# hwang595/ATOMO

Measured on NVIDIA H100. Metric: ResNet-18 CIFAR-10 images/sec (whole box, device-timed, max over ranks), higher is better.
Workload: dtype bf16

## Files before the change

atomo_b200/csrc/bindings.cpp:

```cpp
#include <ATen/cuda/CUDAContext.h>
#include <c10/cuda/CUDAGuard.h>
#include <torch/extension.h>

#include <cstdint>
#include <string>

extern "C" {
const char* atomo_heap_last_error();
int atomo_heap_multicast_supported(int device);
int atomo_heap_posix_fd_supported(int device);
void* atomo_heap_create_vmm(int rank, int world, int device, size_t bytes, const char* job, int want_mc,
                            double timeout_s);
int atomo_heap_mc_phase_a(void* h, double timeout_s);
int atomo_heap_mc_phase_b(void* h);
void* atomo_heap_create_ipc(int rank, int world, int device, size_t bytes, unsigned char* handle_out64);
int atomo_heap_open_ipc(void* h, const unsigned char* all_handles);
uint64_t atomo_heap_ptr(void* h, int rank);
uint64_t atomo_heap_mc_ptr(void* h);
uint64_t atomo_heap_bytes(void* h);
const char* atomo_heap_mode(void* h);
void atomo_heap_destroy(void* h);
void atomo_launch_gram(const float* grad, const void* layers, const void* tiles, int ntiles, float* gpart,
                       cudaStream_t stream);
void atomo_launch_eig_sample(const void* layers, const int* ts_layers, int n_ts, const float* gpart, float* vsel,
                             int* selcount, float* sigma_out, float* ps_arena_peer, long long arena_floats,
                             const void* ctrl, const float* ext_uniforms, int rank, int random_sample,
                             int waterfill, int systematic, int worker_index, int threads, cudaStream_t stream);
void atomo_launch_project_push(const float* grad, const void* layers, const void* tiles, int ntiles,
                               const float* vsel, const int* selcount, float* ps_arena_peer,
                               long long arena_floats, int* push_flag_peer, void* ctrl, int worker_index,
                               int signal, cudaStream_t stream);
void atomo_launch_signal_push(int* push_flag_peer, const void* ctrl, int worker_index, cudaStream_t stream);
int atomo_ps_smem_bytes();
int atomo_ps_tile_elems();
int atomo_ps_max_rows();
int atomo_ps_dense_elems();
int atomo_ps_max_workers();
void atomo_launch_ps_update(const void* layers, const void* tiles, int ntiles, int W, int nflags, int nranks,
                            float* params, float* momentum, float* const* params_peer, float* params_mc,
                            const float* const* grads_peer, const float* grads_mc, const float* arenas,
                            long long arena_floats, int* push_flags, int* const* param_flag_peer, void* ctrl,
                            long long timeout_ticks, float inv_w, int grid, long long* tstats, cudaStream_t stream);
void atomo_launch_wait_params(const int* param_flag, void* ctrl, long long timeout_ticks, long long* tstats,
                              cudaStream_t stream);
void atomo_launch_advance_step(void* ctrl, cudaStream_t stream);
void atomo_launch_param_bcast(const float* src, float* const* params_peer, float* params_mc, int nranks,
                              int self_rank, long long numel, cudaStream_t stream);
void atomo_launch_set_flags(int* const* flag_peer, int nranks, int value, cudaStream_t stream);
long long atomo_bn_partial_floats(long long R, int C);
void atomo_launch_bn_forward(const void* x, const void* res, void* y, long long R, int C, float* acc, float* part,
                             const float* gamma, const float* beta, float* save_mean, float* save_invstd,
                             float* running_mean, float* running_var, float eps, float momentum, int relu,
                             cudaStream_t stream);
void atomo_launch_bn_backward(const void* dy, const void* x, const void* y, void* dx, void* dres, long long R, int C,
                              const float* mean, const float* invstd, const float* gamma, float* acc, float* part,
                              float* dgamma, float* dbeta, int relu, cudaStream_t stream);
int atomo_v2_unit_bytes();
int atomo_v2_ctrl_bytes();
int atomo_v2_enc_smem();
int atomo_v2_ps_smem();
int atomo_v2_ps_tile_elems();
void atomo_v2_launch_encode(const void* units, const void* tiles, int tile0, int ntiles, const long long* gptr,
                            float* gpart, unsigned int* unit_counters, float* vsel, int* selcount, float* sigma_out,
                            float* const* arena_peer, int n_owners, long long arena_floats, void* stage,
                            const void* ctrl, const float* ext_uniforms, float* vprev, int max_sweeps,
                            int random_sample, int waterfill, int systematic, int worker, int resample_empty,
                            int flags, long long* tstats, int group, cudaStream_t stream);
void atomo_v2_launch_project(const void* units, const void* tiles, int tile0, int ntiles, const long long* gptr,
                             const float* vsel, const int* selcount, float* const* arena_peer, int* const* sig_peer,
                             int n_owners, long long arena_floats, int worker, int group, void* ctrl,
                             unsigned int* group_counter, int flags, long long* tstats, int final_group, int timed,
                             cudaStream_t stream);
void atomo_v2_launch_ps(const void* units, const void* tiles, int tile0, int ntiles, int W, int nranks, int group,
                        int final_group, int owner, float* master, float* mom, float* sq, float* sqmax, float* vmom,
                        float* vsq, float* vsqmax, void* wshadow_mc, void* const* wshadow_peer, float* vparams_local,
                        float* vparams_mc, float* const* vparams_peer, const float* vgrads_mc,
                        const float* const* vgrads_peer, const void* const* stage_peer, const float* arenas,
                        long long arena_floats, int* sig, int* const* sig_peer, void* ctrl,
                        unsigned int* group_counter, long long timeout, long long* tstats, float inv_w, int grid,
                        cudaStream_t stream);
void atomo_v2_launch_wait_params(const int* sig, int n_owners, void* ctrl, long long timeout, long long* tstats,
                                 cudaStream_t stream);
void atomo_v2_launch_advance_step(void* ctrl, cudaStream_t stream);
void atomo_v2_launch_bcast_bytes(const void* src, void* const* peer, void* mc, int nranks, int self, long long nbytes,
                                 cudaStream_t stream);
int atomo_gemm_tile_bytes();
int atomo_gemm_smem_bytes();
void atomo_launch_skinny_gemm(const void* tiles, int ntiles, void* ctrl, int grid, cudaStream_t stream);
void atomo_launch_ext_finalize(const void* descs, const void* tiles, int ntiles, const float* arena_y,
                               const float* arena_b, float* ps_arena_peer, long long arena_floats,
                               const void* ctrl, int worker_index, cudaStream_t stream);
int atomo_ext_desc_bytes();
void atomo_launch_qsgd_encode(const float* grad, long long numel, int bucket, int q, int terngrad,
                              const float* clip_ptr, unsigned long long* words_out, float* norms_out,
                              const void* ctrl, int worker_index, const float* ext_uniforms, cudaStream_t stream);
void atomo_launch_qsgd_decode_sum(const unsigned long long* const* words, const float* const* norms, int W,
                                  long long numel, int bucket, int q, int terngrad, float* out_sum,
                                  const int* push_flags, void* ctrl, long long timeout_ticks, cudaStream_t stream);
int atomo_qsgd_max_bucket();
void atomo_launch_entrywise_encode(const float* grad, const void* layers, const void* tiles, int ntiles, float* l1,
                                   int nlayers, float budget, int* idx_out, float* val_out, int* count_out,
                                   int capacity, int* local_count, int* push_flag_peer, void* ctrl,
                                   int worker_index, const float* ext_uniforms, int signal, cudaStream_t stream);
void atomo_launch_entrywise_scatter(const int* const* idx, const float* const* val, const int* const* count, int W,
                                    int capacity, float* out_sum, long long numel, const int* push_flags,
                                    void* ctrl, long long timeout_ticks, cudaStream_t stream);
}

namespace {

inline cudaStream_t cur_stream() { return at::cuda::getCurrentCUDAStream().stream(); }
template <typename T>
inline T* P(uint64_t v) { return reinterpret_cast<T*>(static_cast<uintptr_t>(v)); }

void check_cuda_f32(const torch::Tensor& t, const char* name) {
  TORCH_CHECK(t.is_cuda(), name, " must be a CUDA tensor");
  TORCH_CHECK(t.scalar_type() == torch::kFloat32, name, " must be float32");
  TORCH_CHECK(t.is_contiguous(), name, " must be contiguous");
}

uint64_t heap_create_vmm(int rank, int world, int device, uint64_t bytes, const std::string& job, bool want_mc,
                         double timeout_s) {
  void* h = atomo_heap_create_vmm(rank, world, device, bytes, job.c_str(), want_mc ? 1 : 0, timeout_s);
  return reinterpret_cast<uint64_t>(h);
}
py::tuple heap_create_ipc(int rank, int world, int device, uint64_t bytes) {
  unsigned char handle[64] = {0};
  void* h = atomo_heap_create_ipc(rank, world, device, bytes, handle);
  return py::make_tuple(reinterpret_cast<uint64_t>(h), py::bytes(reinterpret_cast<const char*>(handle), 64));
}
bool heap_open_ipc(uint64_t h, const std::string& all_handles) {
  return atomo_heap_open_ipc(P<void>(h), reinterpret_cast<const unsigned char*>(all_handles.data())) != 0;
}

torch::Tensor tensor_from_ptr(uint64_t ptr, int64_t numel, const std::string& dtype, int device) {
  auto dt = dtype == "int32"      ? torch::kInt32
            : dtype == "int64"    ? torch::kInt64
            : dtype == "uint8"    ? torch::kUInt8
            : dtype == "bfloat16" ? torch::kBFloat16
                                  : torch::kFloat32;
  auto opts = torch::TensorOptions().dtype(dt).device(torch::kCUDA, device);
  return torch::from_blob(P<void>(ptr), {numel}, [](void*) {}, opts);
}

void gram(const torch::Tensor& grad, const torch::Tensor& layers, const torch::Tensor& tiles, int ntiles,
          torch::Tensor gpart) {
  check_cuda_f32(grad, "grad");
  c10::cuda::CUDAGuard guard(grad.device());
  atomo_launch_gram(grad.data_ptr<float>(), layers.data_ptr(), tiles.data_ptr(), ntiles, gpart.data_ptr<float>(),
                    cur_stream());
}

void eig_sample(const torch::Tensor& layers, const torch::Tensor& ts_layers, const torch::Tensor& gpart,
                torch::Tensor vsel, torch::Tensor selcount, c10::optional<torch::Tensor> sigma_out,
                uint64_t ps_arena_peer, int64_t arena_floats, const torch::Tensor& ctrl,
                c10::optional<torch::Tensor> ext_uniforms, int rank, bool random_sample, bool waterfill,
                bool systematic, int worker_index, int threads) {
  c10::cuda::CUDAGuard guard(gpart.device());
  atomo_launch_eig_sample(layers.data_ptr(), ts_layers.data_ptr<int>(), (int)ts_layers.numel(),
                          gpart.data_ptr<float>(), vsel.data_ptr<float>(), selcount.data_ptr<int>(),
                          sigma_out.has_value() ? sigma_out->data_ptr<float>() : nullptr, P<float>(ps_arena_peer),
                          arena_floats, ctrl.data_ptr(),
                          ext_uniforms.has_value() ? ext_uniforms->data_ptr<float>() : nullptr, rank,
                          random_sample, waterfill, systematic, worker_index, threads, cur_stream());
}

void project_push(const torch::Tensor& grad, const torch::Tensor& layers, const torch::Tensor& tiles, int ntiles,
                  const torch::Tensor& vsel, const torch::Tensor& selcount, uint64_t ps_arena_peer,
                  int64_t arena_floats, uint64_t push_flag_peer, torch::Tensor ctrl, int worker_index, bool signal) {
  check_cuda_f32(grad, "grad");
  c10::cuda::CUDAGuard guard(grad.device());
  atomo_launch_project_push(grad.data_ptr<float>(), layers.data_ptr(), tiles.data_ptr(), ntiles,
                            vsel.data_ptr<float>(), selcount.data_ptr<int>(), P<float>(ps_arena_peer), arena_floats,
                            P<int>(push_flag_peer), ctrl.data_ptr(), worker_index, signal ? 1 : 0, cur_stream());
}

void signal_push(uint64_t push_flag_peer, const torch::Tensor& ctrl, int worker_index) {
  c10::cuda::CUDAGuard guard(ctrl.device());
  atomo_launch_signal_push(P<int>(push_flag_peer), ctrl.data_ptr(), worker_index, cur_stream());
}

void check_nhwc_bf16(const torch::Tensor& t, const char* name) {
  TORCH_CHECK(t.is_cuda() && t.scalar_type() == torch::kBFloat16, name, " must be a CUDA bf16 tensor");
  TORCH_CHECK(t.dim() == 4 && t.is_contiguous(at::MemoryFormat::ChannelsLast), name, " must be channels_last");
  TORCH_CHECK(t.size(1) % 8 == 0 && t.size(1) <= 2048, name, ": C must be a multiple of 8 (<= 2048)");
}

void bn_forward(const torch::Tensor& x, c10::optional<torch::Tensor> res, torch::Tensor y, torch::Tensor acc,
                const torch::Tensor& gamma, const torch::Tensor& beta, torch::Tensor save_mean,
                torch::Tensor save_invstd, c10::optional<torch::Tensor> running_mean,
                c10::optional<torch::Tensor> running_var, double eps, double momentum, bool relu) {
  check_nhwc_bf16(x, "x");
  check_nhwc_bf16(y, "y");
  if (res.has_value()) check_nhwc_bf16(*res, "residual");
  c10::cuda::CUDAGuard guard(x.device());
  const long long R = x.numel() / x.size(1);
  auto part = torch::empty({atomo_bn_partial_floats(R, (int)x.size(1))}, acc.options());
  atomo_launch_bn_forward(x.data_ptr(), res.has_value() ? res->data_ptr() : nullptr, y.data_ptr(), R, (int)x.size(1),
                          acc.data_ptr<float>(), part.data_ptr<float>(), gamma.data_ptr<float>(), beta.data_ptr<float>(),
                          save_mean.data_ptr<float>(), save_invstd.data_ptr<float>(),
                          running_mean.has_value() ? running_mean->data_ptr<float>() : nullptr,
                          running_var.has_value() ? running_var->data_ptr<float>() : nullptr, (float)eps,
                          (float)momentum, relu ? 1 : 0, cur_stream());
}

void bn_backward(const torch::Tensor& dy, const torch::Tensor& x, const torch::Tensor& y, torch::Tensor dx,
                 c10::optional<torch::Tensor> dres, const torch::Tensor& mean, const torch::Tensor& invstd,
                 const torch::Tensor& gamma, torch::Tensor acc, torch::Tensor dgamma, torch::Tensor dbeta, bool relu) {
  check_nhwc_bf16(dy, "dy");
  check_nhwc_bf16(x, "x");
  check_nhwc_bf16(dx, "dx");
  c10::cuda::CUDAGuard guard(x.device());
  const long long R = x.numel() / x.size(1);
  auto part = torch::empty({atomo_bn_partial_floats(R, (int)x.size(1))}, acc.options());
  atomo_launch_bn_backward(dy.data_ptr(), x.data_ptr(), y.data_ptr(), dx.data_ptr(),
                           dres.has_value() ? dres->data_ptr() : nullptr, R, (int)x.size(1), mean.data_ptr<float>(),
                           invstd.data_ptr<float>(), gamma.data_ptr<float>(), acc.data_ptr<float>(),
                           part.data_ptr<float>(), dgamma.data_ptr<float>(), dbeta.data_ptr<float>(), relu ? 1 : 0,
                           cur_stream());
}

void skinny_gemm(const torch::Tensor& tiles, int ntiles, torch::Tensor ctrl, int grid) {
  c10::cuda::CUDAGuard guard(tiles.device());
  atomo_launch_skinny_gemm(tiles.data_ptr(), ntiles, ctrl.data_ptr(), grid, cur_stream());
}

void ext_finalize(const torch::Tensor& descs, const torch::Tensor& tiles, int ntiles, const torch::Tensor& arena_y,
                  const torch::Tensor& arena_b, uint64_t ps_arena_peer, int64_t arena_floats,
                  const torch::Tensor& ctrl, int worker_index) {
  check_cuda_f32(arena_y, "arena_y");
  c10::cuda::CUDAGuard guard(arena_y.device());
  atomo_launch_ext_finalize(descs.data_ptr(), tiles.data_ptr(), ntiles, arena_y.data_ptr<float>(),
                            arena_b.data_ptr<float>(), P<float>(ps_arena_peer), arena_floats, ctrl.data_ptr(),
                            worker_index, cur_stream());
}

void ps_update(const torch::Tensor& layers, const torch::Tensor& tiles, int ntiles, int W, int nflags, int nranks,
               torch::Tensor params, torch::Tensor momentum, const torch::Tensor& params_peer, uint64_t params_mc,
               const torch::Tensor& grads_peer, uint64_t grads_mc, uint64_t arenas, int64_t arena_floats,
               uint64_t push_flags, const torch::Tensor& param_flag_peer, torch::Tensor ctrl,
               int64_t timeout_ticks, double inv_w, int grid, uint64_t tstats) {
  check_cuda_f32(params, "params");
  check_cuda_f32(momentum, "momentum");
  TORCH_CHECK(W <= atomo_ps_max_workers(), "too many workers for ps_update");
  c10::cuda::CUDAGuard guard(params.device());
  atomo_launch_ps_update(layers.data_ptr(), tiles.data_ptr(), ntiles, W, nflags, nranks, params.data_ptr<float>(),
                         momentum.data_ptr<float>(), reinterpret_cast<float* const*>(params_peer.data_ptr()),
                         P<float>(params_mc), reinterpret_cast<const float* const*>(grads_peer.data_ptr()),
                         P<const float>(grads_mc), P<const float>(arenas), arena_floats, P<int>(push_flags),
                         reinterpret_cast<int* const*>(param_flag_peer.data_ptr()), ctrl.data_ptr(), timeout_ticks,
                         (float)inv_w, grid, P<long long>(tstats), cur_stream());
}

void wait_params(uint64_t param_flag, torch::Tensor ctrl, int64_t timeout_ticks, uint64_t tstats) {
  c10::cuda::CUDAGuard guard(ctrl.device());
  atomo_launch_wait_params(P<const int>(param_flag), ctrl.data_ptr(), timeout_ticks, P<long long>(tstats),
                           cur_stream());
}
void advance_step(torch::Tensor ctrl) {
  c10::cuda::CUDAGuard guard(ctrl.device());
  atomo_launch_advance_step(ctrl.data_ptr(), cur_stream());
}
void param_bcast(const torch::Tensor& src, const torch::Tensor& params_peer, uint64_t params_mc, int nranks,
                 int self_rank, int64_t numel) {
  check_cuda_f32(src, "src");
  c10::cuda::CUDAGuard guard(src.device());
  atomo_launch_param_bcast(src.data_ptr<float>(), reinterpret_cast<float* const*>(params_peer.data_ptr()),
                           P<float>(params_mc), nranks, self_rank, numel, cur_stream());
}
void set_flags(const torch::Tensor& flag_peer, int nranks, int value) {
  c10::cuda::CUDAGuard guard(flag_peer.device());
  atomo_launch_set_flags(reinterpret_cast<int* const*>(flag_peer.data_ptr()), nranks, value, cur_stream());
}

void qsgd_encode(const torch::Tensor& grad, int64_t numel, int bucket, int q, bool terngrad,
                 c10::optional<torch::Tensor> clip, uint64_t words_out, uint64_t norms_out,
                 const torch::Tensor& ctrl, int worker_index, c10::optional<torch::Tensor> ext_uniforms) {
  check_cuda_f32(grad, "grad");
  TORCH_CHECK(q >= 1 && q <= 14, "GPU QSGD supports quantization_level in [1, 14]");
  TORCH_CHECK(bucket >= 32 && bucket <= atomo_qsgd_max_bucket(), "bucket_size out of range for the GPU path");
  c10::cuda::CUDAGuard guard(grad.device());
  atomo_launch_qsgd_encode(grad.data_ptr<float>(), numel, bucket, q, terngrad,
                           clip.has_value() ? clip->data_ptr<float>() : nullptr, P<unsigned long long>(words_out),
                           P<float>(norms_out), ctrl.data_ptr(), worker_index,
                           ext_uniforms.has_value() ? ext_uniforms->data_ptr<float>() : nullptr, cur_stream());
}
void qsgd_decode_sum(const torch::Tensor& words_ptrs, const torch::Tensor& norms_ptrs, int W, int64_t numel,
                     int bucket, int q, bool terngrad, torch::Tensor out_sum, uint64_t push_flags,
                     torch::Tensor ctrl, int64_t timeout_ticks) {
  check_cuda_f32(out_sum, "out_sum");
  c10::cuda::CUDAGuard guard(out_sum.device());
  atomo_launch_qsgd_decode_sum(reinterpret_cast<const unsigned long long* const*>(words_ptrs.data_ptr()),
                               reinterpret_cast<const float* const*>(norms_ptrs.data_ptr()), W, numel, bucket, q,
                               terngrad, out_sum.data_ptr<float>(), P<const int>(push_flags), ctrl.data_ptr(),
                               timeout_ticks, cur_stream());
}
void entrywise_encode(const torch::Tensor& grad, const torch::Tensor& layers, const torch::Tensor& tiles,
                      int ntiles, torch::Tensor l1, double budget, uint64_t idx_out, uint64_t val_out,
                      uint64_t count_out, int capacity, torch::Tensor local_count, uint64_t push_flag_peer,
                      torch::Tensor ctrl, int worker_index, c10::optional<torch::Tensor> ext_uniforms, bool signal) {
  check_cuda_f32(grad, "grad");
  c10::cuda::CUDAGuard guard(grad.device());
// ... 129 lines not shown
```

atomo_b200/csrc/bn_kernels.cu:

```cuda
#include <cuda_bf16.h>
#include <stdlib.h>

#include "common.cuh"

namespace atomo {

constexpr int BN_THREADS = 256;
constexpr int BN_MAX_C = 2048;

struct bf16x8 {
  uint4 v;
};

__device__ __forceinline__ void unpack8(const uint4 v, float (&f)[8]) {
  const __nv_bfloat162* p = reinterpret_cast<const __nv_bfloat162*>(&v);
#pragma unroll
  for (int i = 0; i < 4; ++i) {
    const float2 t = __bfloat1622float2(p[i]);
    f[2 * i] = t.x;
    f[2 * i + 1] = t.y;
  }
}
__device__ __forceinline__ uint4 pack8(const float (&f)[8]) {
  uint4 v;
  __nv_bfloat162* p = reinterpret_cast<__nv_bfloat162*>(&v);
#pragma unroll
  for (int i = 0; i < 4; ++i) p[i] = __floats2bfloat162_rn(f[2 * i], f[2 * i + 1]);
  return v;
}


__global__ void __launch_bounds__(BN_THREADS)
bn_stats_kernel(const uint4* __restrict__ x, long long R, int C, float* __restrict__ part) {
  extern __shared__ float red[];
  const int CG = C >> 3;
  const int RL = BN_THREADS / CG;
  const int cg = threadIdx.x % CG, rl = threadIdx.x / CG;
  float s[8], q[8];
#pragma unroll
  for (int i = 0; i < 8; ++i) { s[i] = 0.f; q[i] = 0.f; }
  if (rl < RL) {
    const long long stride = (long long)gridDim.x * RL;
    long long r = (long long)blockIdx.x * RL + rl;
    for (; r + 3 * stride < R; r += 4 * stride) {
      uint4 v[4];
#pragma unroll
      for (int k = 0; k < 4; ++k) v[k] = __ldg(x + (r + k * stride) * CG + cg);
#pragma unroll
      for (int k = 0; k < 4; ++k) {
        float f[8];
        unpack8(v[k], f);
#pragma unroll
        for (int i = 0; i < 8; ++i) { s[i] += f[i]; q[i] = fmaf(f[i], f[i], q[i]); }
      }
    }
    for (; r < R; r += stride) {
      float f[8];
      unpack8(__ldg(x + r * CG + cg), f);
#pragma unroll
      for (int i = 0; i < 8; ++i) { s[i] += f[i]; q[i] = fmaf(f[i], f[i], q[i]); }
    }
#pragma unroll
    for (int i = 0; i < 8; ++i) {
      red[rl * C + cg * 8 + i] = s[i];
      red[RL * C + rl * C + cg * 8 + i] = q[i];
    }
  }
  __syncthreads();
  for (int c = threadIdx.x; c < C; c += blockDim.x) {
    float a = 0.f, b = 0.f;
    for (int k = 0; k < RL; ++k) { a += red[k * C + c]; b += red[RL * C + k * C + c]; }
    part[(long long)blockIdx.x * 2 * C + c] = a;
    part[(long long)blockIdx.x * 2 * C + C + c] = b;
  }
}

__global__ void __launch_bounds__(BN_THREADS)
bn_apply_kernel(const uint4* __restrict__ x, const uint4* __restrict__ res, uint4* __restrict__ y, long long R, int C,
                const float* __restrict__ acc, const float* __restrict__ gamma, const float* __restrict__ beta,
                float* __restrict__ save_mean, float* __restrict__ save_invstd, float* __restrict__ running_mean,
                float* __restrict__ running_var, float eps, float momentum, int relu) {
  extern __shared__ float tab[];
  const float invR = 1.f / (float)R;
  for (int c = threadIdx.x; c < C; c += blockDim.x) {
    const float mean = acc[c] * invR;
    const float var = fmaxf(acc[C + c] * invR - mean * mean, 0.f);
    const float invstd = rsqrtf(var + eps);
    const float sc = gamma[c] * invstd;
    tab[c] = sc;
    tab[C + c] = beta[c] - mean * sc;
    if (blockIdx.x == 0) {
      save_mean[c] = mean;
      save_invstd[c] = invstd;
      if (running_mean != nullptr) {
        const float unbiased = R > 1 ? var * (float)R / (float)(R - 1) : var;
        running_mean[c] = (1.f - momentum) * running_mean[c] + momentum * mean;
        running_var[c] = (1.f - momentum) * running_var[c] + momentum * unbiased;
      }
    }
  }
  __syncthreads();
  const int CG = C >> 3;
  const long long total = R * CG;
  for (long long e = (long long)blockIdx.x * blockDim.x + threadIdx.x; e < total; e += (long long)gridDim.x * blockDim.x) {
    const int cg = (int)(e % CG);
    float f[8], o[8];
    unpack8(__ldg(x + e), f);
    if (res != nullptr) {
      float g[8];
      unpack8(__ldg(res + e), g);
#pragma unroll
      for (int i = 0; i < 8; ++i) o[i] = fmaf(f[i], tab[cg * 8 + i], tab[C + cg * 8 + i]) + g[i];
    } else {
#pragma unroll
      for (int i = 0; i < 8; ++i) o[i] = fmaf(f[i], tab[cg * 8 + i], tab[C + cg * 8 + i]);
    }
    if (relu) {
#pragma unroll
      for (int i = 0; i < 8; ++i) o[i] = fmaxf(o[i], 0.f);
    }
    y[e] = pack8(o);
  }
}

__global__ void __launch_bounds__(BN_THREADS)
bn_bwd_reduce_kernel(const uint4* __restrict__ dy, const uint4* __restrict__ x, const uint4* __restrict__ y,
                     long long R, int C, const float* __restrict__ mean, const float* __restrict__ invstd,
                     float* __restrict__ part, int relu) {
  extern __shared__ float red[];
  const int CG = C >> 3;
  const int RL = BN_THREADS / CG;
  const int cg = threadIdx.x % CG, rl = threadIdx.x / CG;
  float s[8], q[8], mu[8], is[8];
#pragma unroll
  for (int i = 0; i < 8; ++i) { s[i] = 0.f; q[i] = 0.f; mu[i] = mean[cg * 8 + i]; is[i] = invstd[cg * 8 + i]; }
  if (rl < RL) {
    const long long stride = (long long)gridDim.x * RL;
    long long r = (long long)blockIdx.x * RL + rl;
    for (; r + stride < R; r += 2 * stride) {
      uint4 dv[2], xq[2], yq[2];
#pragma unroll
      for (int k = 0; k < 2; ++k) {
        dv[k] = __ldg(dy + (r + k * stride) * CG + cg);
        xq[k] = __ldg(x + (r + k * stride) * CG + cg);
        if (relu) yq[k] = __ldg(y + (r + k * stride) * CG + cg);
      }
#pragma unroll
      for (int k = 0; k < 2; ++k) {
        float d[8], xv[8];
        unpack8(dv[k], d);
        unpack8(xq[k], xv);
        if (relu) {
          float yv[8];
          unpack8(yq[k], yv);
#pragma unroll
          for (int i = 0; i < 8; ++i) d[i] = yv[i] > 0.f ? d[i] : 0.f;
        }
#pragma unroll
        for (int i = 0; i < 8; ++i) { s[i] += d[i]; q[i] = fmaf(d[i], (xv[i] - mu[i]) * is[i], q[i]); }
      }
    }
    for (; r < R; r += stride) {
      float d[8], xv[8];
      unpack8(__ldg(dy + r * CG + cg), d);
      unpack8(__ldg(x + r * CG + cg), xv);
      if (relu) {
        float yv[8];
        unpack8(__ldg(y + r * CG + cg), yv);
#pragma unroll
        for (int i = 0; i < 8; ++i) d[i] = yv[i] > 0.f ? d[i] : 0.f;
      }
#pragma unroll
      for (int i = 0; i < 8; ++i) { s[i] += d[i]; q[i] = fmaf(d[i], (xv[i] - mu[i]) * is[i], q[i]); }
    }
#pragma unroll
    for (int i = 0; i < 8; ++i) {
      red[rl * C + cg * 8 + i] = s[i];
      red[RL * C + rl * C + cg * 8 + i] = q[i];
    }
  }
  __syncthreads();
  for (int c = threadIdx.x; c < C; c += blockDim.x) {
    float a = 0.f, b = 0.f;
    for (int k = 0; k < RL; ++k) { a += red[k * C + c]; b += red[RL * C + k * C + c]; }
    part[(long long)blockIdx.x * 2 * C + c] = a;
    part[(long long)blockIdx.x * 2 * C + C + c] = b;
  }
}

__global__ void __launch_bounds__(BN_THREADS)
bn_bwd_apply_kernel(const uint4* __restrict__ dy, const uint4* __restrict__ x, const uint4* __restrict__ y,
                    uint4* __restrict__ dx, uint4* __restrict__ dres, long long R, int C,
                    const float* __restrict__ mean, const float* __restrict__ invstd, const float* __restrict__ gamma,
                    const float* __restrict__ acc, float* __restrict__ dgamma, float* __restrict__ dbeta, int relu) {
  extern __shared__ float tab[];
  const float invR = 1.f / (float)R;
  for (int c = threadIdx.x; c < C; c += blockDim.x) {
    tab[c] = mean[c];
    tab[C + c] = invstd[c];
    tab[2 * C + c] = gamma[c] * invstd[c];
    tab[3 * C + c] = acc[c] * invR;
    tab[4 * C + c] = acc[C + c] * invR;
    if (blockIdx.x == 0) {
      dbeta[c] = acc[c];
      dgamma[c] = acc[C + c];
    }
  }
  __syncthreads();
  const int CG = C >> 3;
  const long long total = R * CG;
  for (long long e = (long long)blockIdx.x * blockDim.x + threadIdx.x; e < total; e += (long long)gridDim.x * blockDim.x) {
    const int c0 = (int)(e % CG) * 8;
    float d[8], xv[8], o[8];
    unpack8(__ldg(dy + e), d);
    unpack8(__ldg(x + e), xv);
    if (relu) {
      float yv[8];
      unpack8(__ldg(y + e), yv);
#pragma unroll
      for (int i = 0; i < 8; ++i) d[i] = yv[i] > 0.f ? d[i] : 0.f;
    }
#pragma unroll
    for (int i = 0; i < 8; ++i) {
      const float xhat = (xv[i] - tab[c0 + i]) * tab[C + c0 + i];
      o[i] = tab[2 * C + c0 + i] * (d[i] - tab[3 * C + c0 + i] - xhat * tab[4 * C + c0 + i]);
    }
    dx[e] = pack8(o);
    if (dres != nullptr) dres[e] = pack8(d);
  }
}

constexpr int BN_SUM_THREADS = 1024;
__global__ void __launch_bounds__(BN_SUM_THREADS)
bn_sum_partials_kernel(const float* __restrict__ part, int P, int W, float* __restrict__ acc) {
  __shared__ float red[BN_SUM_THREADS / 32][32];
  const int lane = threadIdx.x & 31, g = threadIdx.x >> 5;
  const int col = blockIdx.x * 32 + lane;
  float s = 0.f;
  if (col < W) {
#pragma unroll 4
    for (int p = g; p < P; p += BN_SUM_THREADS / 32) s += __ldg(part + (long long)p * W + col);
  }
  red[g][lane] = s;
  __syncthreads();
  if (g == 0 && col < W) {
    float t = red[0][lane];
#pragma unroll
    for (int k = 1; k < BN_SUM_THREADS / 32; ++k) t += red[k][lane];
    acc[col] = t;
  }
}

extern "C" {

static int bn_grid(long long work_items, int per_block) {
  long long g = (work_items + per_block - 1) / per_block;
  if (g > num_sms() * 8) g = num_sms() * 8;
  if (g < 1) g = 1;
  return (int)g;
}
static int g_bn_reduce_ctas = 0;
static int bn_reduce_grid(long long R, int RL) {
  if (g_bn_reduce_ctas == 0) {
    const char* e = getenv("ATOMO_BN_REDUCE_CTAS");
    g_bn_reduce_ctas = e != nullptr ? atoi(e) : 296;
    if (g_bn_reduce_ctas < 1) g_bn_reduce_ctas = 296;
  }
  long long g = (R + RL - 1) / RL;
  if (g > g_bn_reduce_ctas) g = g_bn_reduce_ctas;
  return (int)(g < 1 ? 1 : g);
}

long long atomo_bn_partial_floats(long long R, int C) {
  return (long long)bn_reduce_grid(R, BN_THREADS / (C / 8)) * 2 * C;
}

static void bn_sum_partials(const float* part, int P, int C, float* acc, cudaStream_t stream) {
  bn_sum_partials_kernel<<<(2 * C + 31) / 32, BN_SUM_THREADS, 0, stream>>>(part, P, 2 * C, acc);
}

void atomo_launch_bn_forward(const void* x, const void* res, void* y, long long R, int C, float* acc, float* part,
                             const float* gamma, const float* beta, float* save_mean, float* save_invstd,
                             float* running_mean, float* running_var, float eps, float momentum, int relu,
                             cudaStream_t stream) {
  const int CG = C / 8, RL = BN_THREADS / CG;
  const int g1 = bn_reduce_grid(R, RL);
  bn_stats_kernel<<<g1, BN_THREADS, 2 * RL * C * sizeof(float), stream>>>((const uint4*)x, R, C, part);
  bn_sum_partials(part, g1, C, acc, stream);
  const int g2 = bn_grid(R * CG, BN_THREADS * 2);
  bn_apply_kernel<<<g2, BN_THREADS, 2 * C * sizeof(float), stream>>>((const uint4*)x, (const uint4*)res, (uint4*)y, R,
                                                                     C, acc, gamma, beta, save_mean, save_invstd,
                                                                     running_mean, running_var, eps, momentum, relu);
}

void atomo_launch_bn_backward(const void* dy, const void* x, const void* y, void* dx, void* dres, long long R, int C,
                              const float* mean, const float* invstd, const float* gamma, float* acc, float* part,
                              float* dgamma, float* dbeta, int relu, cudaStream_t stream) {
  const int CG = C / 8, RL = BN_THREADS / CG;
  const int g1 = bn_reduce_grid(R, RL);
  bn_bwd_reduce_kernel<<<g1, BN_THREADS, 2 * RL * C * sizeof(float), stream>>>((const uint4*)dy, (const uint4*)x,
                                                                               (const uint4*)y, R, C, mean, invstd,
                                                                               part, relu);
  bn_sum_partials(part, g1, C, acc, stream);
  const int g2 = bn_grid(R * CG, BN_THREADS * 2);
  bn_bwd_apply_kernel<<<g2, BN_THREADS, 5 * C * sizeof(float), stream>>>((const uint4*)dy, (const uint4*)x,
                                                                         (const uint4*)y, (uint4*)dx, (uint4*)dres, R,
                                                                         C, mean, invstd, gamma, acc, dgamma, dbeta,
                                                                         relu);
}
}
}
```

atomo_b200/ops/fused_bn.py:

```python
from __future__ import annotations

from typing import Optional

import torch
import torch.nn as nn
import torch.nn.functional as F

from ._ext import load as _load


class _FusedBNFn(torch.autograd.Function):
    @staticmethod
    def forward(ctx, x, weight, bias, running_mean, running_var, residual, relu, eps, momentum, acc_fwd, acc_bwd,
                grad_sink=None):
        C = _load()
        y = torch.empty_like(x, memory_format=torch.channels_last)
        nch = x.size(1)
        acc = acc_fwd if acc_fwd is not None else torch.empty(2 * nch, dtype=torch.float32, device=x.device)
        mean = torch.empty(nch, dtype=torch.float32, device=x.device)
        invstd = torch.empty(nch, dtype=torch.float32, device=x.device)
        C.bn_forward(x, residual, y, acc, weight, bias, mean, invstd, running_mean, running_var, eps, momentum, relu)
        ctx.save_for_backward(x, y, weight, mean, invstd)
        ctx.relu = relu
        ctx.has_res = residual is not None
        ctx.acc_bwd = acc_bwd
        ctx.grad_sink = grad_sink
        return y

    @staticmethod
    def backward(ctx, dy):
        C = _load()
        x, y, weight, mean, invstd = ctx.saved_tensors
        if not dy.is_contiguous(memory_format=torch.channels_last):
            dy = dy.contiguous(memory_format=torch.channels_last)
        nch = x.size(1)
        dx = torch.empty_like(x, memory_format=torch.channels_last)
        dres = torch.empty_like(x, memory_format=torch.channels_last) if ctx.has_res else None
        acc = ctx.acc_bwd if ctx.acc_bwd is not None else torch.empty(2 * nch, dtype=torch.float32, device=x.device)
        if ctx.grad_sink is not None:
            dgamma, dbeta = ctx.grad_sink
            C.bn_backward(dy, x, y, dx, dres, mean, invstd, weight, acc, dgamma, dbeta, ctx.relu)
            return dx, None, None, None, None, dres, None, None, None, None, None, None
        dgamma = torch.empty(nch, dtype=torch.float32, device=x.device)
        dbeta = torch.empty(nch, dtype=torch.float32, device=x.device)
        C.bn_backward(dy, x, y, dx, dres, mean, invstd, weight, acc, dgamma, dbeta, ctx.relu)
        return dx, dgamma, dbeta, None, None, dres, None, None, None, None, None, None


class BNAct(nn.BatchNorm2d):

    fused = False
    _acc_fwd = None
    _acc_bwd = None
    _grad_sink = None

    def _can_fuse(self, x: torch.Tensor, residual: Optional[torch.Tensor]) -> bool:
        if not (self.fused and self.training and x.is_cuda and x.dtype == torch.bfloat16 and x.dim() == 4):
            return False
        if x.size(1) % 8 != 0 or x.size(1) > 2048 or not self.track_running_stats or self.momentum is None:
            return False
        if not x.is_contiguous(memory_format=torch.channels_last):
            return False
        if residual is not None and (residual.dtype != x.dtype or residual.shape != x.shape or
                                     not residual.is_contiguous(memory_format=torch.channels_last)):
            return False
        return self.weight is not None and self.weight.dtype == torch.float32

    def forward(self, x: torch.Tensor, residual: Optional[torch.Tensor] = None, relu: bool = False) -> torch.Tensor:
        if self._can_fuse(x, residual):
            return _FusedBNFn.apply(x, self.weight, self.bias, self.running_mean, self.running_var, residual,
                                    relu, self.eps, self.momentum, self._acc_fwd, self._acc_bwd, self._grad_sink)
        out = super().forward(x)
        if residual is not None:
            out = out + residual
        return F.relu(out) if relu else out


def enable_fused_bn(module: nn.Module, enabled: bool = True, arena_device=None):
    mods = [m for m in module.modules() if isinstance(m, BNAct)]
    arena = None
    if enabled and arena_device is not None and mods:
        total = sum(4 * m.num_features for m in mods)
        arena = torch.zeros(total, dtype=torch.float32, device=arena_device)
        off = 0
        for m in mods:
            c2 = 2 * m.num_features
            m._acc_fwd, m._acc_bwd = arena[off:off + c2], arena[off + c2:off + 2 * c2]
            off += 2 * c2
    for m in mods:
        m.fused = enabled
        if arena is None:
            m._acc_fwd = m._acc_bwd = None
    return len(mods), arena
```

atomo_b200/runtime/shadow_engine.py:

```python
from __future__ import annotations

import os
from typing import List, Optional

import numpy as np
import torch
import torch.distributed as dist
import torch.nn as nn

from ..ops import plan2 as P2
from ..ops._ext import load as load_ext
from ..parallel.symm import SymmetricHeap

SIGNAL_INTS = 1024


def _dev_bytes(b: bytes, device) -> torch.Tensor:
    return torch.frombuffer(bytearray(b if len(b) else b"\0" * 16), dtype=torch.uint8).to(device)


class ShadowEngine:
    def __init__(self, model: nn.Module, rank: int = 0, world: int = 1, code: str = "svd", svd_rank: int = 3,
                 lr: float = 0.01, momentum: float = 0.0, weight_decay: float = 0.0, nesterov: bool = False,
                 dampening: float = 0.0, optimizer: str = "sgd", betas=(0.9, 0.999), eps: float = 1e-8,
# ... 242 lines not shown
                        self.gpart.data_ptr(), self.counters.data_ptr(), self.vsel.data_ptr(),
                        self.selcount.data_ptr(), self.sigma.data_ptr(), self.t_arena_peer.data_ptr(), self.n_owners,
                        pl.arena_floats, self.wstage.data_ptr(), self.ctrl.data_ptr(), 0,
                        self.vprev.data_ptr() if self.vprev is not None else 0, self.max_sweeps, self.random_sample,
                        self.waterfill, self.systematic, self.worker_index, self.resample_empty, self.kflags,
                        self.tstats.data_ptr(), g)
            self._nlaunch += 1
        elif nt > 0:
            C.v2_encode(self.t_units.data_ptr(), self.t_enc_tiles.data_ptr(), t0, nt, self.t_gptr.data_ptr(),
                        self.gpart.data_ptr(), self.counters.data_ptr(), self.vsel.data_ptr(),
                        self.selcount.data_ptr(), 0, self.t_arena_peer.data_ptr(), self.n_owners, pl.arena_floats,
                        self.wstage.data_ptr(), self.ctrl.data_ptr(), 0, 0, 0, False, False, False, self.worker_index, False, self.kflags,
                        self.tstats.data_ptr(), g)
            self._nlaunch += 1
        C.v2_project(self.t_units.data_ptr(), self.t_enc_tiles.data_ptr(), t0, nt, self.t_gptr.data_ptr(),
                     self.vsel.data_ptr(), self.selcount.data_ptr(), self.t_arena_peer.data_ptr(),
                     self.t_sig_owner.data_ptr(), self.n_owners, pl.arena_floats, self.worker_index, g,
                     self.ctrl.data_ptr(), self.cnt_enc_group + 4 * g, self.kflags, self.tstats.data_ptr(),
                     self._fired == self.G, nt > 0)
        self._nlaunch += 1

    def _launch_ps(self, g: int, final: bool):
        C, pl = self.C, self.plan
        t0, nt = pl.ps_range[g][self.owner_index]
        p = lambda t: t.data_ptr() if t is not None else 0
        C.v2_ps(self.t_units.data_ptr(), self.t_ps_tiles.data_ptr(), t0, nt, self.W, self.world, g, final,
                self.owner_index, p(self.master), p(self.mom), p(self.sq), p(self.sqmax), p(self.vmom), p(self.vsq),
                p(self.vsqmax), self.wshadow_mc, self.t_wshadow_peer.data_ptr(), self.vparams.data_ptr(),
                self.vparams_mc, self.t_vparams_peer.data_ptr(), self.vgrads_mc, self.t_vgrads_peer.data_ptr(),
                self.t_stage_peer.data_ptr(), self.heap.region_ptr("arena"), pl.arena_floats,
                self.signals.data_ptr(), self.t_sig_all.data_ptr(), self.ctrl.data_ptr(), self.cnt_ps_group + 4 * g,
                self.timeout_ticks, self.tstats.data_ptr(), 1.0 / self.W, max(1, min(self.ps_grid, max(nt, 1))))
        self._nlaunch += 1

    def _launch_group(self, g: int):
        final = self._fired == self.G - 1
        self._fired += 1
        if not self.overlap:
            self._launch_encode(g)
            if self.is_owner:
                self._launch_ps(g, final)
            return
        cur = torch.cuda.current_stream(self.device)
        self.ev_ready[g].record(cur)
        self.s_enc.wait_event(self.ev_ready[g])
        with torch.cuda.stream(self.s_enc):
            if self._jitter_us:
                torch.cuda._sleep(int(self._jitter_rng.uniform(0, self._jitter_us) * 1900))
            self._launch_encode(g)
            self.ev_push[g].record(self.s_enc)
            if final:
                self.ev_enc_done.record(self.s_enc)
        if self.is_owner:
            self.s_ps.wait_event(self.ev_push[g])
            with torch.cuda.stream(self.s_ps):
                if self._jitter_us:
                    torch.cuda._sleep(int(self._jitter_rng.uniform(0, self._jitter_us) * 1900))
                self._launch_ps(g, final)
                if final:
                    self.ev_ps_done.record(self.s_ps)

    def _forward_backward(self):
        x, y = self.static_x, self.static_y
        with torch.autocast("cuda", dtype=torch.bfloat16):
            logits = self.model(x)
            loss = self.criterion(logits.float(), y)
        loss.backward()
        with torch.no_grad():
            lg = logits.detach().float()
            k = min(5, lg.size(1))
            hit = lg.topk(k, 1).indices.eq(y.view(-1, 1))
            self.loss_buf[0] = loss.detach()
            self.loss_buf[1] = hit[:, :1].float().sum() * (100.0 / y.numel())
            self.loss_buf[2] = hit.float().sum() * (100.0 / y.numel())

    def _step_body(self):
        C = self.C
        self._nlaunch = 0
        C.v2_wait_params(self.signals.data_ptr(), self.n_owners, self.ctrl.data_ptr(), self.timeout_ticks,
                         self.tstats.data_ptr())
        self._nlaunch += 1
        if self.is_worker:
            self.vgrads.zero_()
            if self.bn_arena is not None:
                self.bn_arena.zero_()
            for p in self.w_params:
                p.grad = None
            self._pending, self._fired = list(self.group_size), 0
            self._forward_backward()
            self._nlaunch += 4 * self.fused_bn_layers
            assert self._fired == self.G, "a backward group never fired (%d of %d)" % (self._fired, self.G)
            if self.overlap:
                cur = torch.cuda.current_stream(self.device)
                cur.wait_event(self.ev_enc_done)
                if self.is_owner:
                    cur.wait_event(self.ev_ps_done)
        elif self.is_owner:
            for g in range(self.G):
                self._launch_ps(g, g == self.G - 1)
        C.v2_advance_step(self.ctrl.data_ptr())
        self._nlaunch += 1
        self.launches_per_step = self._nlaunch

    def prepare(self, x_example: torch.Tensor, y_example: torch.Tensor, warmup: int = 3):
        self.static_x = torch.empty_like(x_example, device=self.device)
        if self.static_x.dim() == 4:
            self.static_x = self.static_x.contiguous(memory_format=torch.channels_last)
        self.static_y = torch.empty_like(y_example, device=self.device)
        self.static_x.copy_(x_example)
        self.static_y.copy_(y_example)
        self.s_copy = torch.cuda.Stream(device=self.device)
        self.stage_x = [torch.empty_like(self.static_x) for _ in range(2)]
        self.stage_y = [torch.empty_like(self.static_y) for _ in range(2)]
        self._stage_ready = [torch.cuda.Event() for _ in range(2)]
        self._stage_free = [torch.cuda.Event() for _ in range(2)]
        self._stage_i = 0
        self.model.train()
        s = self.s_main
        s.wait_stream(torch.cuda.current_stream(self.device))
        with torch.cuda.stream(s):
            for _ in range(warmup):
                self._step_body()
                self.step += 1
        torch.cuda.current_stream(self.device).wait_stream(s)
        torch.cuda.synchronize(self.device)
        if self.use_graph:
            self.graph = torch.cuda.CUDAGraph()
            self._capturing = True
            try:
                with torch.cuda.graph(self.graph, stream=self.s_main):
                    self._step_body()
            finally:
                self._capturing = False
            self.t_gptr.copy_(torch.from_numpy(self.host_gptr.copy()))
            torch.cuda.synchronize(self.device)
        return self

    def train_step(self, x: Optional[torch.Tensor] = None, y: Optional[torch.Tensor] = None):
        if x is not None and self.is_worker:
            if x.is_cuda:
                self.static_x.copy_(x, non_blocking=True)
                self.static_y.copy_(y, non_blocking=True)
            else:
                k = self._stage_i
                self._stage_i ^= 1
                cur = torch.cuda.current_stream(self.device)
                with torch.cuda.stream(self.s_copy):
                    self.s_copy.wait_event(self._stage_free[k])
                    self.stage_x[k].copy_(x, non_blocking=True)
                    self.stage_y[k].copy_(y, non_blocking=True)
                    self._stage_ready[k].record(self.s_copy)
                cur.wait_event(self._stage_ready[k])
                self.static_x.copy_(self.stage_x[k], non_blocking=True)
                self.static_y.copy_(self.stage_y[k], non_blocking=True)
                self._stage_free[k].record(cur)
        if self.graph is not None:
            self.graph.replay()
        else:
            self._step_body()
        self.step += 1
        return self.loss_buf

    def _owned_mask(self):
        pl = self.plan
        mw = torch.zeros(pl.w_total, dtype=torch.float32, device=self.device)
        mv = torch.zeros(pl.v_total, dtype=torch.float32, device=self.device)
        if not self.is_owner:
            return mw, mv
# ... 125 lines not shown
```

Baseline: 47300.

## Save bit-packed ReLU mask and chain fused BN kernels with PDL

The fused BN+ReLU forward now writes a one-bit-per-element uint8 mask alongside its output. Backward reads this mask instead of the bf16 output tensor y, which cuts backward read traffic and means y no longer has to be kept alive for autograd. The stats, sum-partials, apply and backward kernels are launched with programmatic dependent launch (griddepcontrol wait and launch_dependents) so each kernel's prologue can overlap the tail of the previous one. The per-step zeroing of the BN accumulator arena is also dropped. The forward pass pays an extra mask write, and dropping the zeroing depends on the accumulators being fully overwritten, which looks true since sum_partials stores into acc directly.

Measured after the change: 49080 (median of 6 runs). +3.8%, better.

```diff
diff --git a/atomo_b200/csrc/bindings.cpp b/atomo_b200/csrc/bindings.cpp
--- a/atomo_b200/csrc/bindings.cpp
+++ b/atomo_b200/csrc/bindings.cpp
@@ -48,13 +48,12 @@
                               int self_rank, long long numel, cudaStream_t stream);
 void atomo_launch_set_flags(int* const* flag_peer, int nranks, int value, cudaStream_t stream);
 long long atomo_bn_partial_floats(long long R, int C);
-void atomo_launch_bn_forward(const void* x, const void* res, void* y, long long R, int C, float* acc, float* part,
-                             const float* gamma, const float* beta, float* save_mean, float* save_invstd,
-                             float* running_mean, float* running_var, float eps, float momentum, int relu,
-                             cudaStream_t stream);
-void atomo_launch_bn_backward(const void* dy, const void* x, const void* y, void* dx, void* dres, long long R, int C,
+void atomo_launch_bn_forward(const void* x, const void* res, void* y, void* mask, long long R, int C, float* acc,
+                             float* part, const float* gamma, const float* beta, float* save_mean, float* save_invstd,
+                             float* running_mean, float* running_var, float eps, float momentum, cudaStream_t stream);
+void atomo_launch_bn_backward(const void* dy, const void* x, const void* mask, void* dx, void* dres, long long R, int C,
                               const float* mean, const float* invstd, const float* gamma, float* acc, float* part,
-                              float* dgamma, float* dbeta, int relu, cudaStream_t stream);
+                              float* dgamma, float* dbeta, cudaStream_t stream);
 int atomo_v2_unit_bytes();
 int atomo_v2_ctrl_bytes();
 int atomo_v2_enc_smem();
@@ -186,38 +185,49 @@
   TORCH_CHECK(t.size(1) % 8 == 0 && t.size(1) <= 2048, name, ": C must be a multiple of 8 (<= 2048)");
 }
 
-void bn_forward(const torch::Tensor& x, c10::optional<torch::Tensor> res, torch::Tensor y, torch::Tensor acc,
-                const torch::Tensor& gamma, const torch::Tensor& beta, torch::Tensor save_mean,
-                torch::Tensor save_invstd, c10::optional<torch::Tensor> running_mean,
-                c10::optional<torch::Tensor> running_var, double eps, double momentum, bool relu) {
+void check_relu_mask(const torch::Tensor& mask, const torch::Tensor& x) {
+  TORCH_CHECK(mask.is_cuda() && mask.scalar_type() == torch::kUInt8 && mask.is_contiguous(),
+              "mask must be a contiguous CUDA uint8 tensor");
+  TORCH_CHECK(mask.numel() == x.numel() / 8, "mask must hold numel(x) / 8 bytes");
+}
+
+void bn_forward(const torch::Tensor& x, c10::optional<torch::Tensor> res, torch::Tensor y,
+                c10::optional<torch::Tensor> mask, torch::Tensor acc, const torch::Tensor& gamma,
+                const torch::Tensor& beta, torch::Tensor save_mean, torch::Tensor save_invstd,
+                c10::optional<torch::Tensor> running_mean, c10::optional<torch::Tensor> running_var, double eps,
+                double momentum) {
   check_nhwc_bf16(x, "x");
   check_nhwc_bf16(y, "y");
   if (res.has_value()) check_nhwc_bf16(*res, "residual");
+  if (mask.has_value()) check_relu_mask(*mask, x);
   c10::cuda::CUDAGuard guard(x.device());
   const long long R = x.numel() / x.size(1);
   auto part = torch::empty({atomo_bn_partial_floats(R, (int)x.size(1))}, acc.options());
-  atomo_launch_bn_forward(x.data_ptr(), res.has_value() ? res->data_ptr() : nullptr, y.data_ptr(), R, (int)x.size(1),
-                          acc.data_ptr<float>(), part.data_ptr<float>(), gamma.data_ptr<float>(), beta.data_ptr<float>(),
+  atomo_launch_bn_forward(x.data_ptr(), res.has_value() ? res->data_ptr() : nullptr, y.data_ptr(),
+                          mask.has_value() ? mask->data_ptr() : nullptr, R, (int)x.size(1), acc.data_ptr<float>(),
+                          part.data_ptr<float>(), gamma.data_ptr<float>(), beta.data_ptr<float>(),
                           save_mean.data_ptr<float>(), save_invstd.data_ptr<float>(),
                           running_mean.has_value() ? running_mean->data_ptr<float>() : nullptr,
                           running_var.has_value() ? running_var->data_ptr<float>() : nullptr, (float)eps,
-                          (float)momentum, relu ? 1 : 0, cur_stream());
-}
-
-void bn_backward(const torch::Tensor& dy, const torch::Tensor& x, const torch::Tensor& y, torch::Tensor dx,
+                          (float)momentum, cur_stream());
+  C10_CUDA_KERNEL_LAUNCH_CHECK();
+}
+
+void bn_backward(const torch::Tensor& dy, const torch::Tensor& x, c10::optional<torch::Tensor> mask, torch::Tensor dx,
                  c10::optional<torch::Tensor> dres, const torch::Tensor& mean, const torch::Tensor& invstd,
-                 const torch::Tensor& gamma, torch::Tensor acc, torch::Tensor dgamma, torch::Tensor dbeta, bool relu) {
+                 const torch::Tensor& gamma, torch::Tensor acc, torch::Tensor dgamma, torch::Tensor dbeta) {
   check_nhwc_bf16(dy, "dy");
   check_nhwc_bf16(x, "x");
   check_nhwc_bf16(dx, "dx");
+  if (mask.has_value()) check_relu_mask(*mask, x);
   c10::cuda::CUDAGuard guard(x.device());
   const long long R = x.numel() / x.size(1);
   auto part = torch::empty({atomo_bn_partial_floats(R, (int)x.size(1))}, acc.options());
-  atomo_launch_bn_backward(dy.data_ptr(), x.data_ptr(), y.data_ptr(), dx.data_ptr(),
+  atomo_launch_bn_backward(dy.data_ptr(), x.data_ptr(), mask.has_value() ? mask->data_ptr() : nullptr, dx.data_ptr(),
                            dres.has_value() ? dres->data_ptr() : nullptr, R, (int)x.size(1), mean.data_ptr<float>(),
                            invstd.data_ptr<float>(), gamma.data_ptr<float>(), acc.data_ptr<float>(),
-                           part.data_ptr<float>(), dgamma.data_ptr<float>(), dbeta.data_ptr<float>(), relu ? 1 : 0,
-                           cur_stream());
+                           part.data_ptr<float>(), dgamma.data_ptr<float>(), dbeta.data_ptr<float>(), cur_stream());
+  C10_CUDA_KERNEL_LAUNCH_CHECK();
 }
 
 void skinny_gemm(const torch::Tensor& tiles, int ntiles, torch::Tensor ctrl, int grid) {
diff --git a/atomo_b200/csrc/bn_kernels.cu b/atomo_b200/csrc/bn_kernels.cu
--- a/atomo_b200/csrc/bn_kernels.cu
+++ b/atomo_b200/csrc/bn_kernels.cu
@@ -28,6 +28,9 @@
   for (int i = 0; i < 4; ++i) p[i] = __floats2bfloat162_rn(f[2 * i], f[2 * i + 1]);
   return v;
 }
+
+__device__ __forceinline__ void pdl_wait() { asm volatile("griddepcontrol.wait;" ::: "memory"); }
+__device__ __forceinline__ void pdl_launch_dependents() { asm volatile("griddepcontrol.launch_dependents;"); }
 
 
 __global__ void __launch_bounds__(BN_THREADS)
@@ -66,6 +69,7 @@
       red[RL * C + rl * C + cg * 8 + i] = q[i];
     }
   }
+  pdl_launch_dependents();
   __syncthreads();
   for (int c = threadIdx.x; c < C; c += blockDim.x) {
     float a = 0.f, b = 0.f;
@@ -76,11 +80,13 @@
 }
 
 __global__ void __launch_bounds__(BN_THREADS)
-bn_apply_kernel(const uint4* __restrict__ x, const uint4* __restrict__ res, uint4* __restrict__ y, long long R, int C,
-                const float* __restrict__ acc, const float* __restrict__ gamma, const float* __restrict__ beta,
-                float* __restrict__ save_mean, float* __restrict__ save_invstd, float* __restrict__ running_mean,
-                float* __restrict__ running_var, float eps, float momentum, int relu) {
+bn_apply_kernel(const uint4* __restrict__ x, const uint4* __restrict__ res, uint4* __restrict__ y,
+                uint8_t* __restrict__ mask, long long R, int C, const float* __restrict__ acc,
+                const float* __restrict__ gamma, const float* __restrict__ beta, float* __restrict__ save_mean,
+                float* __restrict__ save_invstd, float* __restrict__ running_mean, float* __restrict__ running_var,
+                float eps, float momentum, int relu) {
   extern __shared__ float tab[];
+  pdl_wait();
   const float invR = 1.f / (float)R;
   for (int c = threadIdx.x; c < C; c += blockDim.x) {
     const float mean = acc[c] * invR;
@@ -119,12 +125,21 @@
 #pragma unroll
       for (int i = 0; i < 8; ++i) o[i] = fmaxf(o[i], 0.f);
     }
-    y[e] = pack8(o);
+    const uint4 out = pack8(o);
+    y[e] = out;
+    if (relu) {
+      float yv[8];
+      unpack8(out, yv);
+      unsigned m = 0;
+#pragma unroll
+      for (int i = 0; i < 8; ++i) m |= (yv[i] > 0.f ? 1u : 0u) << i;
+      mask[e] = (uint8_t)m;
+    }
   }
 }
 
 __global__ void __launch_bounds__(BN_THREADS)
-bn_bwd_reduce_kernel(const uint4* __restrict__ dy, const uint4* __restrict__ x, const uint4* __restrict__ y,
+bn_bwd_reduce_kernel(const uint4* __restrict__ dy, const uint4* __restrict__ x, const uint8_t* __restrict__ mask,
                      long long R, int C, const float* __restrict__ mean, const float* __restrict__ invstd,
                      float* __restrict__ part, int relu) {
   extern __shared__ float red[];
@@ -138,12 +153,13 @@
     const long long stride = (long long)gridDim.x * RL;
     long long r = (long long)blockIdx.x * RL + rl;
     for (; r + stride < R; r += 2 * stride) {
-      uint4 dv[2], xq[2], yq[2];
+      uint4 dv[2], xq[2];
+      unsigned mq[2];
 #pragma unroll
       for (int k = 0; k < 2; ++k) {
         dv[k] = __ldg(dy + (r + k * stride) * CG + cg);
         xq[k] = __ldg(x + (r + k * stride) * CG + cg);
-        if (relu) yq[k] = __ldg(y + (r + k * stride) * CG + cg);
+        if (relu) mq[k] = __ldg(mask + (r + k * stride) * CG + cg);
       }
 #pragma unroll
       for (int k = 0; k < 2; ++k) {
@@ -151,10 +167,8 @@
         unpack8(dv[k], d);
         unpack8(xq[k], xv);
         if (relu) {
-          float yv[8];
-          unpack8(yq[k], yv);
-#pragma unroll
-          for (int i = 0; i < 8; ++i) d[i] = yv[i] > 0.f ? d[i] : 0.f;
+#pragma unroll
+          for (int i = 0; i < 8; ++i) d[i] = (mq[k] >> i) & 1u ? d[i] : 0.f;
         }
 #pragma unroll
         for (int i = 0; i < 8; ++i) { s[i] += d[i]; q[i] = fmaf(d[i], (xv[i] - mu[i]) * is[i], q[i]); }
@@ -165,10 +179,9 @@
       unpack8(__ldg(dy + r * CG + cg), d);
       unpack8(__ldg(x + r * CG + cg), xv);
       if (relu) {
-        float yv[8];
-        unpack8(__ldg(y + r * CG + cg), yv);
-#pragma unroll
-        for (int i = 0; i < 8; ++i) d[i] = yv[i] > 0.f ? d[i] : 0.f;
+        const unsigned m = __ldg(mask + r * CG + cg);
+#pragma unroll
+        for (int i = 0; i < 8; ++i) d[i] = (m >> i) & 1u ? d[i] : 0.f;
       }
 #pragma unroll
       for (int i = 0; i < 8; ++i) { s[i] += d[i]; q[i] = fmaf(d[i], (xv[i] - mu[i]) * is[i], q[i]); }
@@ -179,6 +192,7 @@
       red[RL * C + rl * C + cg * 8 + i] = q[i];
     }
   }
+  pdl_launch_dependents();
   __syncthreads();
   for (int c = threadIdx.x; c < C; c += blockDim.x) {
     float a = 0.f, b = 0.f;
@@ -189,11 +203,12 @@
 }
 
 __global__ void __launch_bounds__(BN_THREADS)
-bn_bwd_apply_kernel(const uint4* __restrict__ dy, const uint4* __restrict__ x, const uint4* __restrict__ y,
+bn_bwd_apply_kernel(const uint4* __restrict__ dy, const uint4* __restrict__ x, const uint8_t* __restrict__ mask,
                     uint4* __restrict__ dx, uint4* __restrict__ dres, long long R, int C,
                     const float* __restrict__ mean, const float* __restrict__ invstd, const float* __restrict__ gamma,
                     const float* __restrict__ acc, float* __restrict__ dgamma, float* __restrict__ dbeta, int relu) {
   extern __shared__ float tab[];
+  pdl_wait();
   const float invR = 1.f / (float)R;
   for (int c = threadIdx.x; c < C; c += blockDim.x) {
     tab[c] = mean[c];
@@ -215,10 +230,9 @@
     unpack8(__ldg(dy + e), d);
     unpack8(__ldg(x + e), xv);
     if (relu) {
-      float yv[8];
-      unpack8(__ldg(y + e), yv);
-#pragma unroll
-      for (int i = 0; i < 8; ++i) d[i] = yv[i] > 0.f ? d[i] : 0.f;
+      const unsigned m = __ldg(mask + e);
+#pragma unroll
+      for (int i = 0; i < 8; ++i) d[i] = (m >> i) & 1u ? d[i] : 0.f;
     }
 #pragma unroll
     for (int i = 0; i < 8; ++i) {
@@ -237,10 +251,12 @@
   const int lane = threadIdx.x & 31, g = threadIdx.x >> 5;
   const int col = blockIdx.x * 32 + lane;
   float s = 0.f;
+  pdl_wait();
   if (col < W) {
 #pragma unroll 4
     for (int p = g; p < P; p += BN_SUM_THREADS / 32) s += __ldg(part + (long long)p * W + col);
   }
+  pdl_launch_dependents();
   red[g][lane] = s;
   __syncthreads();
   if (g == 0 && col < W) {
@@ -249,6 +265,22 @@
     for (int k = 1; k < BN_SUM_THREADS / 32; ++k) t += red[k][lane];
     acc[col] = t;
   }
+}
+
+template <typename... Params, typename... Args>
+static void launch_pdl(void (*kernel)(Params...), int grid, int block, size_t smem, cudaStream_t stream,
+                       Args... args) {
+  cudaLaunchAttribute attr[1];
+  attr[0].id = cudaLaunchAttributeProgrammaticStreamSerialization;
+  attr[0].val.programmaticStreamSerializationAllowed = 1;
+  cudaLaunchConfig_t cfg = {};
+  cfg.gridDim = dim3(grid);
+  cfg.blockDim = dim3(block);
+  cfg.dynamicSmemBytes = smem;
+  cfg.stream = stream;
+  cfg.attrs = attr;
+  cfg.numAttrs = 1;
+  cudaLaunchKernelEx(&cfg, kernel, args...);
 }
 
 extern "C" {
@@ -276,37 +308,36 @@
 }
 
 static void bn_sum_partials(const float* part, int P, int C, float* acc, cudaStream_t stream) {
-  bn_sum_partials_kernel<<<(2 * C + 31) / 32, BN_SUM_THREADS, 0, stream>>>(part, P, 2 * C, acc);
-}
-
-void atomo_launch_bn_forward(const void* x, const void* res, void* y, long long R, int C, float* acc, float* part,
-                             const float* gamma, const float* beta, float* save_mean, float* save_invstd,
-                             float* running_mean, float* running_var, float eps, float momentum, int relu,
-                             cudaStream_t stream) {
+  launch_pdl(bn_sum_partials_kernel, (2 * C + 31) / 32, BN_SUM_THREADS, 0, stream, part, P, 2 * C, acc);
+}
+
+void atomo_launch_bn_forward(const void* x, const void* res, void* y, void* mask, long long R, int C, float* acc,
+                             float* part, const float* gamma, const float* beta, float* save_mean, float* save_invstd,
+                             float* running_mean, float* running_var, float eps, float momentum, cudaStream_t stream) {
   const int CG = C / 8, RL = BN_THREADS / CG;
   const int g1 = bn_reduce_grid(R, RL);
   bn_stats_kernel<<<g1, BN_THREADS, 2 * RL * C * sizeof(float), stream>>>((const uint4*)x, R, C, part);
   bn_sum_partials(part, g1, C, acc, stream);
   const int g2 = bn_grid(R * CG, BN_THREADS * 2);
-  bn_apply_kernel<<<g2, BN_THREADS, 2 * C * sizeof(float), stream>>>((const uint4*)x, (const uint4*)res, (uint4*)y, R,
-                                                                     C, acc, gamma, beta, save_mean, save_invstd,
-                                                                     running_mean, running_var, eps, momentum, relu);
-}
-
-void atomo_launch_bn_backward(const void* dy, const void* x, const void* y, void* dx, void* dres, long long R, int C,
+  launch_pdl(bn_apply_kernel, g2, BN_THREADS, 2 * C * sizeof(float), stream, (const uint4*)x, (const uint4*)res,
+             (uint4*)y, (uint8_t*)mask, R, C, (const float*)acc, gamma, beta, save_mean, save_invstd, running_mean,
+             running_var, eps, momentum, mask != nullptr ? 1 : 0);
+}
+
+void atomo_launch_bn_backward(const void* dy, const void* x, const void* mask, void* dx, void* dres, long long R, int C,
                               const float* mean, const float* invstd, const float* gamma, float* acc, float* part,
-                              float* dgamma, float* dbeta, int relu, cudaStream_t stream) {
+                              float* dgamma, float* dbeta, cudaStream_t stream) {
   const int CG = C / 8, RL = BN_THREADS / CG;
+  const int relu = mask != nullptr ? 1 : 0;
   const int g1 = bn_reduce_grid(R, RL);
   bn_bwd_reduce_kernel<<<g1, BN_THREADS, 2 * RL * C * sizeof(float), stream>>>((const uint4*)dy, (const uint4*)x,
-                                                                               (const uint4*)y, R, C, mean, invstd,
-                                                                               part, relu);
+                                                                               (const uint8_t*)mask, R, C, mean,
+                                                                               invstd, part, relu);
   bn_sum_partials(part, g1, C, acc, stream);
   const int g2 = bn_grid(R * CG, BN_THREADS * 2);
-  bn_bwd_apply_kernel<<<g2, BN_THREADS, 5 * C * sizeof(float), stream>>>((const uint4*)dy, (const uint4*)x,
-                                                                         (const uint4*)y, (uint4*)dx, (uint4*)dres, R,
-                                                                         C, mean, invstd, gamma, acc, dgamma, dbeta,
-                                                                         relu);
-}
-}
-}
+  launch_pdl(bn_bwd_apply_kernel, g2, BN_THREADS, 5 * C * sizeof(float), stream, (const uint4*)dy, (const uint4*)x,
+             (const uint8_t*)mask, (uint4*)dx, (uint4*)dres, R, C, mean, invstd, gamma, (const float*)acc, dgamma,
+             dbeta, relu);
+}
+}
+}
diff --git a/atomo_b200/ops/fused_bn.py b/atomo_b200/ops/fused_bn.py
--- a/atomo_b200/ops/fused_bn.py
+++ b/atomo_b200/ops/fused_bn.py
@@ -19,9 +19,9 @@
         acc = acc_fwd if acc_fwd is not None else torch.empty(2 * nch, dtype=torch.float32, device=x.device)
         mean = torch.empty(nch, dtype=torch.float32, device=x.device)
         invstd = torch.empty(nch, dtype=torch.float32, device=x.device)
-        C.bn_forward(x, residual, y, acc, weight, bias, mean, invstd, running_mean, running_var, eps, momentum, relu)
-        ctx.save_for_backward(x, y, weight, mean, invstd)
-        ctx.relu = relu
+        mask = torch.empty(x.numel() // 8, dtype=torch.uint8, device=x.device) if relu else None
+        C.bn_forward(x, residual, y, mask, acc, weight, bias, mean, invstd, running_mean, running_var, eps, momentum)
+        ctx.save_for_backward(x, mask, weight, mean, invstd)
         ctx.has_res = residual is not None
         ctx.acc_bwd = acc_bwd
         ctx.grad_sink = grad_sink
@@ -30,7 +30,7 @@
     @staticmethod
     def backward(ctx, dy):
         C = _load()
-        x, y, weight, mean, invstd = ctx.saved_tensors
+        x, mask, weight, mean, invstd = ctx.saved_tensors
         if not dy.is_contiguous(memory_format=torch.channels_last):
             dy = dy.contiguous(memory_format=torch.channels_last)
         nch = x.size(1)
@@ -39,11 +39,11 @@
         acc = ctx.acc_bwd if ctx.acc_bwd is not None else torch.empty(2 * nch, dtype=torch.float32, device=x.device)
         if ctx.grad_sink is not None:
             dgamma, dbeta = ctx.grad_sink
-            C.bn_backward(dy, x, y, dx, dres, mean, invstd, weight, acc, dgamma, dbeta, ctx.relu)
+            C.bn_backward(dy, x, mask, dx, dres, mean, invstd, weight, acc, dgamma, dbeta)
             return dx, None, None, None, None, dres, None, None, None, None, None, None
         dgamma = torch.empty(nch, dtype=torch.float32, device=x.device)
         dbeta = torch.empty(nch, dtype=torch.float32, device=x.device)
-        C.bn_backward(dy, x, y, dx, dres, mean, invstd, weight, acc, dgamma, dbeta, ctx.relu)
+        C.bn_backward(dy, x, mask, dx, dres, mean, invstd, weight, acc, dgamma, dbeta)
         return dx, dgamma, dbeta, None, None, dres, None, None, None, None, None, None
 
 
diff --git a/atomo_b200/runtime/shadow_engine.py b/atomo_b200/runtime/shadow_engine.py
--- a/atomo_b200/runtime/shadow_engine.py
+++ b/atomo_b200/runtime/shadow_engine.py
@@ -348,8 +348,6 @@
         self._nlaunch += 1
         if self.is_worker:
             self.vgrads.zero_()
-            if self.bn_arena is not None:
-                self.bn_arena.zero_()
             for p in self.w_params:
                 p.grad = None
             self._pending, self._fired = list(self.group_size), 0
```
